# anonymousauthors001/SGS-GNN

Hardware: AMD Instinct MI355X
Metric: sampled edges/sec + training steps/sec, Reddit hybrid 20% sparsity (higher is better)
Workload: dtype f32

## Files before the change

include/sgs_hip.h:

```cpp
#ifndef SGS_HIP_H_
#define SGS_HIP_H_

#include <stddef.h>
#include <stdint.h>

#ifdef __cplusplus
extern "C" {
#endif

#define SGS_ABI_VERSION 1

#define SGS_OK 0
#define SGS_EINVAL (-1)
#define SGS_EWORKSPACE (-2)
#define SGS_EHIP (-3)

typedef void* sgs_stream_t;

int sgs_abi_version(void);
const char* sgs_last_error(void);

int sgs_rng_set_epoch_buffer(const uint64_t* epoch_dev);
int sgs_exp_noise(uint64_t seed, uint64_t stream_id, int64_t E, float* noise, sgs_stream_t stream);
int sgs_dropout_keep(uint64_t seed, uint32_t site, int64_t rows, int64_t cols, float p, uint8_t* keep,
// ... 365 lines not shown
                      const int64_t* edge_index, float* dw, void* ws, size_t ws_bytes, sgs_stream_t stream);
int sgs_cheb_spmm(int64_t K, const float* X, int64_t ldx, int64_t N, int64_t D, int64_t nnz, const int32_t* ptr, const int32_t* col,
                  const float* val, float alpha, const float* add, int64_t ldadd, const float* sub, int64_t ldsub, const float* bias, int act,
                  float p_drop, uint64_t seed, uint32_t site, float* Y, int64_t ldy, float* Y2, int64_t ldy2, float scale2,
                  sgs_stream_t stream);

size_t sgs_gemm_tn_workspace_bytes(int64_t K, int64_t M, int64_t N);
int sgs_gemm_tn(const float* A, const float* B, int64_t K, int64_t M, int64_t N, float* C, void* ws, size_t ws_bytes,
                sgs_stream_t stream);
void sgs_gemm_tn_set_tall_variant(int variant);
int sgs_gemm_tn_can_colsum(int64_t K, int64_t M, int64_t N);
int sgs_gemm_tn_colsum(const float* A, const float* B, int64_t K, int64_t M, int64_t N, float* C, float* colsum_A, void* ws,
                       size_t ws_bytes, sgs_stream_t stream);
int sgs_gemm_tn_ld(const float* A, const float* B, int64_t K, int64_t M, int64_t N, float* C, int64_t ldc, float* colsum_A, void* ws,
                   size_t ws_bytes, sgs_stream_t stream);

int sgs_er_weight(const int64_t* edge_index, int64_t E, int64_t N, const int32_t* out_ptr, const int32_t* out_dst, int walk_lengths,
                  int walks, uint64_t seed, float* weight, sgs_stream_t stream);

int sgs_adam_max_tensors(void);
int sgs_adam_step(const int64_t* desc_host, int64_t n_tensors, float lr, float beta1, float beta2, float eps, float weight_decay,
                  int maximize, uint32_t* ticket, sgs_stream_t stream);
int sgs_adam_multi_max_tensors(void);
int sgs_adam_step_multi(const int64_t* desc_host, const float* hyper_host, int64_t n_tensors, uint32_t* ticket, float* loss_sum, const float* loss,
                        uint64_t* epoch, sgs_stream_t stream);

size_t sgs_sample_topq_multi_workspace_bytes(int64_t E, int64_t D);
int sgs_sample_topq_multi(int mode, const float* p, const float* prior, double degree_bias_coef, const float* noise, uint64_t seed,
                          uint64_t stream_id0, int64_t D, int64_t E, int64_t q, const int64_t* edge_index, uint8_t* mask, int64_t* sampled_eid,
                          int64_t* sampled_edge_index, float* stats, float* st_weights, void* ws, size_t ws_bytes, sgs_stream_t stream);
// ... 35 lines not shown
```

sgs-gnn_amd/csrc/gemm_tn.hip:

```cpp
#include "sgs_common.h"

namespace sgs {
namespace {

using f32x16 = __attribute__((ext_vector_type(16))) float;
constexpr int kUnroll = 8;

__global__ void __launch_bounds__(64) gemm_tn_tile(const float* __restrict__ A, const float* __restrict__ B, int64_t K, int M, int N,
                                                  int ksplit, float* __restrict__ slab) {
    const int lane = threadIdx.x, kh = lane >> 5, l31 = lane & 31;
    const int ti = blockIdx.x, tj = blockIdx.y, s = blockIdx.z;
    const int i = ti * 32 + l31, j = tj * 32 + l31;
    const bool iok = i < M, jok = j < N;
    const int64_t per = ((K + ksplit - 1) / ksplit + 1) & ~int64_t(1);
    const int64_t k0 = s * per, k1 = (k0 + per < K) ? k0 + per : K;
    f32x16 acc;
#pragma unroll
    for (int r = 0; r < 16; ++r) acc[r] = 0.f;
    int64_t k = k0;
    for (; k + 2 * kUnroll <= k1; k += 2 * kUnroll) {
        float a[kUnroll], b[kUnroll];
#pragma unroll
        for (int u = 0; u < kUnroll; ++u) {
            const int64_t kk = k + 2 * u + kh;
// ... 9 lines not shown
        const float b = (jok && kk < k1) ? B[kk * N + j] : 0.f;
        acc = __builtin_amdgcn_mfma_f32_32x32x2f32(a, b, acc, 0, 0, 0);
    }
    float* out = slab + static_cast<int64_t>(s) * M * N;
    if (jok) {
#pragma unroll
        for (int r = 0; r < 16; ++r) {
            const int row = ti * 32 + (r & 3) + 8 * (r >> 2) + 4 * kh;
            if (row < M) out[static_cast<int64_t>(row) * N + j] = acc[r];
        }
    }
}

constexpr int kWgUnroll = 8;
template <int NW>
__global__ void __launch_bounds__(64 * NW) gemm_tn_wg(const float* __restrict__ A, const float* __restrict__ B, int64_t K, int M, int N,
                                                     float* __restrict__ C, int64_t ldc) {
    __shared__ float red[NW][16][64];
    const int lane = threadIdx.x & 63, s = threadIdx.x >> 6, kh = lane >> 5, l31 = lane & 31;
    const int ti = blockIdx.x, tj = blockIdx.y;
    const int i = ti * 32 + l31, j = tj * 32 + l31;
    const bool iok = i < M, jok = j < N;
    const int64_t per = ((K + NW - 1) / NW + 1) & ~int64_t(1);
    const int64_t k0 = s * per, k1 = (k0 + per < K) ? k0 + per : K;
    f32x16 acc;
#pragma unroll
    for (int r = 0; r < 16; ++r) acc[r] = 0.f;
    int64_t k = k0;
    for (; k + 2 * kWgUnroll <= k1; k += 2 * kWgUnroll) {
        float a[kWgUnroll], b[kWgUnroll];
#pragma unroll
        for (int u = 0; u < kWgUnroll; ++u) {
            const int64_t kk = k + 2 * u + kh;
            a[u] = iok ? A[kk * M + i] : 0.f;
            b[u] = jok ? B[kk * N + j] : 0.f;
// ... 9 lines not shown
    }
#pragma unroll
    for (int r = 0; r < 16; ++r) red[s][r][lane] = acc[r];
    __syncthreads();
    if (!jok) return;
    constexpr int RPW = 16 / NW;
#pragma unroll
    for (int q = 0; q < RPW; ++q) {
        const int r = s * RPW + q;
        float sum = 0.f;
#pragma unroll
        for (int z = 0; z < NW; ++z) sum += red[z][r][lane];
        const int row = ti * 32 + (r & 3) + 8 * (r >> 2) + 4 * kh;
        if (row < M) C[static_cast<int64_t>(row) * ldc + j] = sum;
    }
}

__global__ void __launch_bounds__(256) gemm_tn_reduce(const float* __restrict__ slab, int64_t mn, int ksplit, float* __restrict__ C,
                                                      const float* __restrict__ cpart = nullptr, int M = 0, float* __restrict__ colsum = nullptr,
                                                      int N = 0, int64_t ldc = 0, const float* __restrict__ rowscale = nullptr,
                                                      float scale = 1.f, const float* __restrict__ dzpart = nullptr, int nz = 0,
                                                      float* __restrict__ dzsum = nullptr, float* __restrict__ Craw = nullptr,
                                                      float* __restrict__ csraw = nullptr, int csplit = 0) {
    const int64_t i = static_cast<int64_t>(blockIdx.x) * 256 + threadIdx.x;
    if (i >= mn) {
        const int64_t c = i - mn;
        if (dzsum && c == M) {
            float acc = 0.f;
            for (int z = 0; z < nz; ++z) acc += dzpart[z];
            dzsum[0] = acc;
// ... 643 lines not shown
inline int pick_ksplit_tall(int64_t K, int64_t M, int64_t N) {
    const int64_t tiles = cdiv(M, 128) * cdiv(N, 64);
    int ks = 1;
    while (ks < 512 && tiles * ks < 1024 && K / (ks * 2) >= 256) ks *= 2;
    return ks;
}

inline int pick_ksplit(int64_t K, int64_t M, int64_t N) {
    if (use_tall(K, M, N)) return pick_ksplit_tall(K, M, N);
    const int64_t tiles = cdiv(M, 32) * cdiv(N, 32);
    int ks = 1;
    while (ks < 64 && tiles * ks < 1024 && K / (ks * 2) >= 64) ks *= 2;
    return ks;
}

}
}

using namespace sgs;

extern "C" {

size_t sgs_gemm_tn_workspace_bytes(int64_t K, int64_t M, int64_t N) {
    if (K < 0 || M < 0 || N < 0) return 256;
    const size_t ks = static_cast<size_t>(pick_ksplit(K, M, N));
    return carve_bytes(ks * M * N, 4) + carve_bytes(ks * M, 4) + carve_bytes(kMaskfeatMaxSlabs * 8 * M + kMaskfeatMaxSlabs, 4) + 512;
}

static int gemm_tn_impl(const float* A, const float* B, int64_t K, int64_t M, int64_t N, float* C, float* colsum_A, void* ws,
                        size_t ws_bytes, hipStream_t stream, int64_t ldc = 0, const uint32_t* Abits = nullptr, const float* dz = nullptr,
// ... 176 lines not shown
        static bool raised = false;
        if (!raised) {
            SGS_HIP_OK(hipFuncSetAttribute(reinterpret_cast<const void*>(&gemm_tn_tall_bf16x6<NW>), hipFuncAttributeMaxDynamicSharedMemorySize,
                                           static_cast<int>(lds)));
            raised = true;
        }
        n_slabs = ks / NW;
        hipLaunchKernelGGL((gemm_tn_tall_bf16x6<NW>), dim3(cdiv(M, 128), cdiv(N, 64), n_slabs), dim3(64 * NW), lds, stream, A, B, K,
                           static_cast<int>(M), static_cast<int>(N), ks, slab, colsum_A ? cpart : static_cast<float*>(nullptr));
    } else if (use_tall(K, M, N) && g_tall_bf16x6)
        hipLaunchKernelGGL((gemm_tn_tall_bf16x6<1>), dim3(cdiv(M, 128), cdiv(N, 64), ks), dim3(64), 0, stream, A, B, K, static_cast<int>(M),
                           static_cast<int>(N), ks, dst, colsum_A ? cpart : static_cast<float*>(nullptr));
    else if (use_tall(K, M, N))
        hipLaunchKernelGGL(gemm_tn_tall_tile, dim3(cdiv(M, 128), cdiv(N, 64), ks), dim3(64), 0, stream, A, B, K, static_cast<int>(M),
                           static_cast<int>(N), ks, dst, colsum_A ? cpart : static_cast<float*>(nullptr));
    else if (ks == 2 || ks == 4 || ks == 8) {
        const dim3 grid(cdiv(M, 32), cdiv(N, 32));
        const int64_t ld = ldc > 0 ? ldc : N;
        if (ks == 8 && K >= 512)
            hipLaunchKernelGGL((gemm_tn_wg<16>), grid, dim3(1024), 0, stream, A, B, K, static_cast<int>(M), static_cast<int>(N), C, ld);
        else if (ks == 8) hipLaunchKernelGGL((gemm_tn_wg<8>), grid, dim3(512), 0, stream, A, B, K, static_cast<int>(M), static_cast<int>(N), C, ld);
        else if (ks == 4) hipLaunchKernelGGL((gemm_tn_wg<4>), grid, dim3(256), 0, stream, A, B, K, static_cast<int>(M), static_cast<int>(N), C, ld);
        else              hipLaunchKernelGGL((gemm_tn_wg<2>), grid, dim3(128), 0, stream, A, B, K, static_cast<int>(M), static_cast<int>(N), C, ld);
        SGS_LAUNCH_OK();
        return SGS_OK;
    } else
        hipLaunchKernelGGL(gemm_tn_tile, dim3(cdiv(M, 32), cdiv(N, 32), ks), dim3(64), 0, stream, A, B, K, static_cast<int>(M),
                           static_cast<int>(N), ks, dst);
    if (ks > 1 || strided)
        hipLaunchKernelGGL(gemm_tn_reduce, dim3(cdiv(M * N + (colsum_A ? M : 0), 256)), dim3(256), 0, stream, slab, M * N, n_slabs, C,
                           static_cast<const float*>(colsum_A ? cpart : nullptr), static_cast<int>(M), colsum_A, static_cast<int>(N), ldc);
    SGS_LAUNCH_OK();
    return SGS_OK;
}

}
```

sgs-gnn_amd/ops.py:

```python
from __future__ import annotations

import os

import numpy as np
import torch

from . import _lib

SAMPLE_LEARNED, SAMPLE_PRIOR = 0, 1
ACT_NONE, ACT_RELU, ACT_RELU_DROPOUT = 0, 1, 2

_workspaces = {}
_retired_workspaces = []
_pin_workspaces = False


def _need_gpu(*tensors):
    for t in tensors:
        if t is not None and not t.is_cuda:
            raise RuntimeError("sgs_gnn_amd: the SGS hot path runs only on a HIP device (got a CPU tensor); "
                               "there is no CPU fallback")


def _ptr(t, dtype=None):
# ... 88 lines not shown

def memo_scope() -> int:
    return _memo_scope


def new_memo_scope() -> int:
    global _memo_scope
    _memo_scope += 1
    return _memo_scope


def drop_memos(module) -> None:
    for mod in module.modules():
        if getattr(mod, "_lin_cache", None) is not None:
            mod._lin_cache = None


_rng_epoch = None


def set_rng_epoch_buffer(epoch) -> None:
    global _rng_epoch
    L = _lib.lib()
    if epoch is not None:
        _need_gpu(epoch)
        if epoch.dtype != torch.int64 or epoch.numel() != 1:
            raise RuntimeError("sgs_gnn_amd: the RNG epoch buffer is one int64 device word")
    _lib.check(L.sgs_rng_set_epoch_buffer(None if epoch is None else epoch.data_ptr()), "sgs_rng_set_epoch_buffer")
    _rng_epoch = epoch

# ... 602 lines not shown
                       "sgs_gemm_tn_ld")
            db1 = _colsum(dv)
        dw2 = _colsum(hdz)
        db2 = _colsum(dz.view(n, 1)).reshape(1)
        if H % 4 == 0:
            dcodes = torch.empty(N, H, dtype=torch.float32, device=dev)
            dU = torch.empty(N, H, dtype=torch.float32, device=dev)
            _lib.check(L.sgs_endpoint_reduce_pair(_ptr(dfeat), _ptr(dv), _ptr(codes), N, H, graph.n_edges, _ptr(graph.in_ptr), _ptr(graph.in_src),
                                                  _ptr(graph.in_eid), _ptr(graph.out_ptr), _ptr(graph.out_dst), _ptr(graph.out_eid),
                                                  _ptr(dcodes), _ptr(dU), _stream()), "sgs_endpoint_reduce_pair")
        else:
            dcodes = _endpoint_reduce(dfeat, dfeat, codes, graph, 1.0, 1.0, H)
            dU = _endpoint_reduce(dv, dv, None, graph, 1.0, -1.0, H)
        if ctx.needs_input_grad[0]:
            dcodes.addmm_(dU, W1[:, H:])
        wsb = workspace(L.sgs_gemm_tn_workspace_bytes(N, H, H), dev)
        _lib.check(L.sgs_gemm_tn_ld(_ptr(dU), _ptr(codes), N, H, H, dW1.data_ptr() + 4 * H, 2 * H, None, wsb.data_ptr(), wsb.numel(), _stream()),
                   "sgs_gemm_tn_ld")
        return dcodes, dW1, db1, dw2, db2, None, None, None, None, None, None, None, None


def _variant_overrides_are_default() -> bool:
    L = _lib.lib()
    return L.sgs_edge_score_get_variant() < 0 and L.sgs_edge_score_get_bwd_variant() < 0


def _edge_score_backward_mask(ctx, L, codes, U, W1, b1, w2, b2, edge_index, eid, graph, n, gp_act, kept=()):
    N, H = codes.shape
    E = edge_index.shape[1]
    dev = codes.device
    f32 = dict(dtype=torch.float32, device=dev)
    p = ctx.p
    bits = torch.empty(n, H // 32, dtype=torch.int32, device=dev)
# ... 25 lines not shown
    scale = float(np.float32(1.0) / (np.float32(1.0) - np.float32(p)))
    wsg = workspace(L.sgs_gemm_tn_workspace_bytes(n, H, H), dev)
    db2 = torch.empty(1, **f32)
    _lib.check((L.sgs_gemm_tn_mask_bf16 if bf16 else L.sgs_gemm_tn_mask)(_ptr(bits), _ptr(dz), _ptr(w2), scale, _ptr(feat), n, H, H, _ptr(dW1), 2 * H, _ptr(db1), _ptr(db2), _ptr(Traw),
                                  _ptr(craw), wsg.data_ptr(), wsg.numel(), _stream()), "sgs_gemm_tn_mask")
    dw2 = _colsum(hdz) if hdz is not None else None
    dcodes = torch.empty(N, H, **f32)
    dU = torch.empty(N, H, **f32)
    _lib.check(L.sgs_endpoint_reduce_pair_bits(_ptr(dfeat), _ptr(bits), _ptr(dz), _ptr(w2), p, _ptr(codes), N, H, graph.n_edges, _ptr(graph.in_ptr),
                                               _ptr(graph.in_src), _ptr(graph.in_eid), _ptr(graph.out_ptr), _ptr(graph.out_dst),
                                               _ptr(graph.out_eid), _ptr(dcodes), _ptr(dU), _ptr(Rraw), _stream()), "sgs_endpoint_reduce_pair_bits")
    if dw2 is None:
        dw2 = torch.empty(H, **f32)
        _lib.check(L.sgs_edge_score_dw2_from_parts(_ptr(W1), _ptr(Traw), _ptr(U), _ptr(Rraw), _ptr(b1), _ptr(craw), N, H, p, _ptr(dw2), _stream()),
                   "sgs_edge_score_dw2_from_parts")
    return _edge_score_backward_mask_tail(L, codes, W1, dcodes, dU, dW1, db1, dw2, db2)


def _edge_score_backward_fused(ctx, L, codes, U, W1, b1, w2, edge_index, eid, graph, n, gp_act, kept, bits, dz):
    N, H = codes.shape
    E = edge_index.shape[1]
    dev = codes.device
    f32 = dict(dtype=torch.float32, device=dev)
    p = ctx.p
    maskbits, p_out = kept
    sd = torch.empty(n, 2, dtype=torch.int32, device=dev)
    wsd = workspace(L.sgs_edge_score_workspace_bytes(0, H, 0), dev)
    bf16 = getattr(ctx, "bf16", False)
    _lib.check((L.sgs_edge_score_bwd_prep_sd_pack_bf16 if bf16 else L.sgs_edge_score_bwd_prep_sd_pack)(_ptr(codes), N, H, _ptr(edge_index), E, _ptr(eid), n, _ptr(gp_act), _ptr(p_out), _ptr(maskbits),
                                                 _ptr(dz), _ptr(bits), _ptr(sd), _ptr(W1), _ptr(w2), p, wsd.data_ptr(), wsd.numel(), _stream()),
               "sgs_edge_score_bwd_prep_sd_pack")
# ... 3 lines not shown
                                                       wsd.numel(), _stream()), "sgs_edge_score_bwd_dfeat_fused_packed")
    dW1 = torch.empty_like(W1)
    db1, db2 = torch.empty(H, **f32), torch.empty(1, **f32)
    Traw, craw, Rraw = torch.empty(H, H, **f32), torch.empty(H, **f32), torch.empty(N, H, **f32)
    scale = float(np.float32(1.0) / (np.float32(1.0) - np.float32(p)))
    wsg = workspace(L.sgs_gemm_tn_workspace_bytes(n, H, H), dev)
    _lib.check((L.sgs_gemm_tn_mask_gather_bf16 if bf16 else L.sgs_gemm_tn_mask_gather)(_ptr(bits), _ptr(dz), _ptr(w2), scale, _ptr(codes), N, _ptr(sd), n, H, H, _ptr(dW1), 2 * H, _ptr(db1), _ptr(db2),
                                         _ptr(Traw), _ptr(craw), wsg.data_ptr(), wsg.numel(), _stream()), "sgs_gemm_tn_mask_gather")
    dcodes, dU = torch.empty(N, H, **f32), torch.empty(N, H, **f32)
    _lib.check(L.sgs_edge_score_bwd_reduce_fused(_ptr(G), _ptr(opart), _ptr(bits), _ptr(dz), _ptr(w2), p, N, H, graph.n_edges, _ptr(graph.in_ptr),
                                                 _ptr(graph.in_eid), _ptr(graph.out_ptr), _ptr(dcodes), _ptr(dU), _ptr(Rraw), _stream()),
               "sgs_edge_score_bwd_reduce_fused")
    dw2 = torch.empty(H, **f32)
    _lib.check(L.sgs_edge_score_dw2_from_parts(_ptr(W1), _ptr(Traw), _ptr(U), _ptr(Rraw), _ptr(b1), _ptr(craw), N, H, p, _ptr(dw2), _stream()),
               "sgs_edge_score_dw2_from_parts")
    return _edge_score_backward_mask_tail(L, codes, W1, dcodes, dU, dW1, db1, dw2, db2)


def _edge_score_backward_mask_tail(L, codes, W1, dcodes, dU, dW1, db1, dw2, db2):
    N, H = codes.shape
    dcodes.addmm_(dU, W1[:, H:])
    wsb = workspace(L.sgs_gemm_tn_workspace_bytes(N, H, H), codes.device)
    _lib.check(L.sgs_gemm_tn_ld(_ptr(dU), _ptr(codes), N, H, H, dW1.data_ptr() + 4 * H, 2 * H, None, wsb.data_ptr(), wsb.numel(), _stream()),
               "sgs_gemm_tn_ld")
    return dcodes, dW1, db1, dw2, db2, None, None, None, None, None, None, None, None


_EdgeScore._backward_mask = staticmethod(_edge_score_backward_mask)


def edge_score(codes, fc1_w, fc1_b, fc2_w, fc2_b, edge_index, active=None, p=0.0, seed=0, site=0, edge_id_offset=0, pairs="cached",
               precision=None):
    precision = _precision if precision is None else check_precision(precision)
    _need_gpu(codes, fc1_w, edge_index)
    if isinstance(pairs, str):
        pairs = get_pairs(edge_index, codes.shape[0])
    return _EdgeScore.apply(codes.contiguous(), fc1_w.contiguous(), fc1_b.contiguous(), fc2_w.reshape(-1).contiguous(), fc2_b.contiguous(),
                            edge_index.contiguous(), active, float(p), int(seed), int(site), int(edge_id_offset), pairs, precision)

# ... 731 lines not shown

    @staticmethod
    def forward(ctx, x, W):
        ctx.save_for_backward(x, W)
        return x @ W.t()

    @staticmethod
    def backward(ctx, dY):
        L = _lib.lib()
        x, W = ctx.saved_tensors
        dx = dW = None
        dY = dY.contiguous()
        if ctx.needs_input_grad[0]:
            dx = dY @ W
        if ctx.needs_input_grad[1]:
            K, M, N = x.shape[0], W.shape[0], W.shape[1]
            dW = torch.empty(M, N, dtype=torch.float32, device=x.device)
            ws = workspace(L.sgs_gemm_tn_workspace_bytes(K, M, N), x.device)
            _lib.check(L.sgs_gemm_tn(_ptr(dY, torch.float32), _ptr(x.contiguous(), torch.float32), K, M, N, _ptr(dW), ws.data_ptr(),
                                     ws.numel(), _stream()), "sgs_gemm_tn")
        return dx, dW


def linear_nobias(x, W):
    _need_gpu(x, W)
    return _LinearNoBias.apply(x, W)


def mean_norm(graph: Graph) -> Norm:
    L = _lib.lib()
    dev = graph.edge_index.device
    nm = Norm()
    nm.graph, nm.w, nm.handle, nm.dis, nm.loopw, nm.what_loop = graph, None, None, None, None, None
    ne = max(graph.n_edges, 1)
    nm.what_in = torch.empty(ne, dtype=torch.float32, device=dev)
# ... 77 lines not shown
    try:
        x._sgs_fcsr = (fc, x._version)
    except Exception:
        pass
    return fc


def _x_wt(x, W):
    fc = feature_csr(x)
    if fc is None:
        return x @ W.t()
    Wt = W.t().contiguous()
    return _spmm(Wt, fc.ptr, fc.col, fc.val, None, None, ACT_NONE, 0.0, 0, 0, fc.N, W.shape[0], fc.nnz)


def _dyt_x(dY, x, W_shape):
    L = _lib.lib()
    fc = feature_csr(x)
    M, Nn = W_shape
    if fc is not None:
        dWt = _spmm(dY.contiguous(), fc.tptr, fc.trow, fc.tval, None, None, ACT_NONE, 0.0, 0, 0, fc.F, M, fc.nnz)
        return dWt.t().contiguous()
    K = x.shape[0]
    dW = torch.empty(M, Nn, dtype=torch.float32, device=x.device)
    ws = workspace(L.sgs_gemm_tn_workspace_bytes(K, M, Nn), x.device)
    _lib.check(L.sgs_gemm_tn(_ptr(dY, torch.float32), _ptr(x.contiguous(), torch.float32), K, M, Nn, _ptr(dW), ws.data_ptr(), ws.numel(), _stream()),
               "sgs_gemm_tn")
    return dW


class _GCNLayer(torch.autograd.Function):

    @staticmethod
    def forward(ctx, x, W, handle, bias, nm, act, p, seed, site, xl):
        gr = nm.graph
        if xl is None:
            xl = _x_wt(x, W)
        N, D = xl.shape
        Y = _spmm(xl, gr.in_ptr, gr.in_src, nm.what_in, nm.what_loop, bias, act, p, seed, site, N, D, gr.n_edges)
        ctx.nm, ctx.act, ctx.p = nm, act, p
        ctx.has_bias, ctx.has_handle = bias is not None, handle is not None
        ctx.save_for_backward(x, W, xl, Y if act != ACT_NONE else None)
        ctx.mark_non_differentiable(xl)
# ... 8 lines not shown
        N, D = xl.shape
        dY = dY.contiguous()
        dx = dW = g = dbias = None
        want_db = ctx.has_bias and ctx.needs_input_grad[3]
        if ctx.act != ACT_NONE and want_db:
            dZ, dbias = _act_bwd_colsum(dY, Y, ctx.act, ctx.p)
        elif ctx.act != ACT_NONE:
            dZ = torch.empty_like(dY)
            _lib.check(L.sgs_act_bwd(_ptr(dY), _ptr(Y), dY.numel(), ctx.act, float(ctx.p), _ptr(dZ), _stream()), "sgs_act_bwd")
        else:
            dZ = dY
        need_x, need_W = ctx.needs_input_grad[0], ctx.needs_input_grad[1]
        if need_x or need_W:
            dxl = _spmm(dZ, gr.out_ptr, gr.out_dst, nm.what_out, nm.what_loop, None, ACT_NONE, 0.0, 0, 0, N, D, gr.n_edges)
            if need_W:
                dW = _dyt_x(dxl, x, W.shape)
            if need_x:
                dx = dxl @ W
        if ctx.has_handle and ctx.needs_input_grad[2]:
            g = torch.empty(gr.n_edges + gr.N, dtype=torch.float32, device=dY.device)
            gw, gl = g[:gr.n_edges], g[gr.n_edges:]
            _lib.check(L.sgs_sddmm_csr(_ptr(dZ), _ptr(xl), N, D, gr.n_edges, _ptr(gr.in_ptr), _ptr(gr.in_src), _ptr(gr.in_eid),
                                       gw.data_ptr(), gl.data_ptr(), _stream()), "sgs_sddmm_csr")
        if want_db and dbias is None:
            dbias = _colsum(dZ)
        return dx, dW, (_handle_grad(nm, g) if g is not None else None), dbias, None, None, None, None, None, None


def gcn_layer(x, W, bias, nm: Norm, act=ACT_NONE, p=0.0, seed=0, site=0, xl=None):
    _need_gpu(x, W, bias)
    if x.dtype != torch.float32 or x.dim() != 2 or x.shape[0] != nm.graph.N:
# ... 54 lines not shown
            return gg

        want_1 = need_x or need_W1 or need_b1 or need_g
        dxl2 = dZ1 = None
        if want_1 or need_W2:
            dxl2 = torch.empty(N, C, **f32)
            if ctx.fused:
                dZ1 = torch.empty(N, H, **f32) if want_1 else None
                db2 = torch.empty(C, **f32) if need_b2 else None
                _lib.check(L.sgs_spmm_csr_bwd_prev(_ptr(dZ2), N, C, gr.n_edges, _ptr(gr.out_ptr), _ptr(gr.out_dst), _ptr(nm.what_out),
                                                   _ptr(nm.what_loop), _ptr(W2 if want_1 else None, torch.float32), H, _ptr(h), ctx.act,
                                                   float(ctx.p), _ptr(dxl2), _ptr(dZ1), _ptr(db2), _stream()), "sgs_spmm_csr_bwd_prev")
            else:
                dxl2 = _spmm(dZ2, gr.out_ptr, gr.out_dst, nm.what_out, nm.what_loop, None, ACT_NONE, 0.0, 0, 0, N, C, gr.n_edges)
        if need_W2:
            dW2 = _dyt_x(dxl2, h, W2.shape)
        if want_1 and not ctx.fused:
            dZ1h = dxl2 @ W2
            if need_b1:
                dZ1, db1 = _act_bwd_colsum(dZ1h, h, ctx.act, ctx.p)
            else:
                dZ1 = torch.empty_like(dZ1h)
                _lib.check(L.sgs_act_bwd(_ptr(dZ1h), _ptr(h), dZ1h.numel(), ctx.act, float(ctx.p), _ptr(dZ1), _stream()), "sgs_act_bwd")
        g2 = sddmm(dZ2, xl2, C) if need_g else None
        if need_b2 and db2 is None:
            db2 = _colsum(dZ2)
        if need_x or need_W1 or (need_b1 and db1 is None and ctx.fused):
            if ctx.fused:
                dxl1 = torch.empty(N, H, **f32)
                db1 = torch.empty(H, **f32) if need_b1 else None
                _lib.check(L.sgs_spmm_csr_bwd_prev(_ptr(dZ1), N, H, gr.n_edges, _ptr(gr.out_ptr), _ptr(gr.out_dst), _ptr(nm.what_out),
                                                   _ptr(nm.what_loop), None, 0, None, ACT_NONE, 0.0, _ptr(dxl1), None, _ptr(db1), _stream()),
                           "sgs_spmm_csr_bwd_prev")
            else:
                dxl1 = _spmm(dZ1, gr.out_ptr, gr.out_dst, nm.what_out, nm.what_loop, None, ACT_NONE, 0.0, 0, 0, N, H, gr.n_edges)
            if need_W1:
                dW1 = _dyt_x(dxl1, x, W1.shape)
            if need_x:
                dx = dxl1 @ W1
        g1 = sddmm(dZ1, xl1, H) if need_g else None
        if need_b1 and db1 is None:
            db1 = _colsum(dZ1)
        if need_g:
            r2, r1 = _handle_grad(nm, g2), _handle_grad(nm, g1)
            g = r2 if r1 is None else (r1 if r2 is None else r2 + r1)
        return dx, dW1, db1, dW2, db2, g, None, None, None, None, None, None


def gcn2(x, W1, b1, W2, b2, nm: Norm, act=ACT_RELU, p=0.0, seed=0, site=0, xl1=None):
    _need_gpu(x, W1, b1, W2, b2)
    if x.dtype != torch.float32 or x.dim() != 2 or x.shape[0] != nm.graph.N:
        raise RuntimeError("gcn2: x must be float32 [N, F]")
# ... 481 lines not shown
```

sgs-gnn_amd/stepgraph.py:

```python
from __future__ import annotations

import ctypes
import gc
import os
import time

import torch

from . import _lib, ops
from .data import Batch

_DEBUG = os.environ.get("SGS_SG_DEBUG", "")
_PREFETCH = os.environ.get("SGS_SG_PREFETCH", "1") != "0"
_E_ALIGN = 2048


def _capturable(opt) -> bool:
    return all(bool(g.get("capturable", False)) for g in opt.param_groups)


def _opt_signature(optimizers):
    if optimizers is None:
        return None
    sig = []
# ... 392 lines not shown
            cur.wait_stream(self.stream)
            torch.cuda.synchronize()
            ops.workspace_handover(self.device)
            self.capture_seconds += time.perf_counter() - t0
            self.captures += 1
            if was_enabled:
                gc.enable()

    def _warm_up(self, slot: _Slot) -> None:
        from .training import _ce, learned_loss, sampled_forward
        b, a = slot.batch, self.args
        ops.drop_memos(self.model)
        ops.new_memo_scope()
        with torch.cuda.stream(self.stream):
            if not slot.sampled:
                _ce(self.criterion, self.model(b, b.edge_index), b).backward()
            else:
                st = sampled_forward(self.pipeline, a, self.model, b, self.q, self.use_checkpoint)
                if st.random_out is not None:
                    _ce(self.criterion, st.random_out, b).backward(retain_graph=True)
                    self._clear_grads()
                learned_loss(a, self.criterion, st, b).backward()
        self._clear_grads()
        torch.cuda.synchronize()

    def _capture_segments(self, c: _Slot) -> None:
        from .training import _ce, learned_loss, sampled_forward, sampled_prefix
        if not self._epoch_started:
            self.epoch_word.fill_(1)
            self.host_epoch = 1
            self._epoch_started = True
        a, batch = self.args, c.batch
        self._clear_grads()
        torch.cuda.synchronize()
        c.g1 = torch.cuda.CUDAGraph()
        ops.drop_memos(self.model)
        ops.new_memo_scope()
        if self.dp and self.g3 is None:
            self._capture_g3()
        if not c.sampled:
            if self.dp:
                self._bind_bucket()
            with torch.cuda.graph(c.g1, stream=self.stream, capture_error_mode=self.capture_mode):
                if self.dp:
                    self.sync.flat.zero_()
                out = self.model(batch, batch.edge_index)
                c.loss = _ce(self.criterion, out, batch)
                c.loss.backward(gradient=self.one)
                self._steps_and_tick((self.optimizers[1],) if (self.optimizers is not None and not self.dp) else (), c.loss)
            c.grads = self._grads()
            c.loss = c.loss.detach()
            self._clear_grads()
            return
        pre, pool = None, None
        if (a.conditional or a.sparse_edge_mlp) and _DEBUG != "fork":
            c.g0 = torch.cuda.CUDAGraph()
            ops.set_rng_epoch_buffer(self.epoch_pre)
            try:
                with ops.workspace_slot(1), torch.cuda.graph(c.g0, stream=self.stream, capture_error_mode=self.capture_mode):
                    pre = sampled_prefix(a, batch, self.q)
            finally:
                ops.set_rng_epoch_buffer(self.epoch_word)
            pool = c.g0.pool()
# ... 3 lines not shown
                                 prefix=pre, gate_publish=(self.epoch_word, self.host_gate))
        pool = c.g1.pool()
        c.cbuf = st.cbuf
        if self.debug_keep:
            c.keep = dict(rsei=st.rsei, eid=st.smp.eid, sampled_edge_index=st.sampled_edge_index,
                          edge_probs_full=st.edge_probs_full.detach(), w=st.edge_probs_for_loss.detach(),
                          learned_out=st.learned_out.detach(),
                          random_out=None if st.random_out is None else st.random_out.detach())
        c.g2l = torch.cuda.CUDAGraph()
        if self.dp:
            self._bind_bucket()
        with torch.cuda.graph(c.g2l, stream=self.stream, pool=pool, capture_error_mode=self.capture_mode):
            if self.dp:
                self.sync.flat.zero_()
            loss_l = learned_loss(a, self.criterion, st, batch)
            loss_l.backward(gradient=self.one, retain_graph=st.random_out is not None)
            if self.dp:
                self.sync.flag.fill_(1.0)
            self._steps_and_tick(tuple(self.optimizers) if (self.optimizers is not None and not self.dp) else (), loss_l)
        c.grads_l = self._grads()
        c.loss_l = loss_l.detach()
        self._clear_grads()
        c.g2r = None
        if st.random_out is not None:
            c.g2r = torch.cuda.CUDAGraph()
            if self.dp:
                self._bind_bucket()
            with torch.cuda.graph(c.g2r, stream=self.stream, pool=pool, capture_error_mode=self.capture_mode):
                if self.dp:
                    self.sync.flat.zero_()
                loss_r = _ce(self.criterion, st.random_out, batch)
                loss_r.backward(gradient=self.one)
                self._steps_and_tick((self.optimizers[1],) if (self.optimizers is not None and not self.dp) else (), loss_r)
            c.grads_r = self._grads()
            c.loss_r = loss_r.detach()
            self._clear_grads()

    def _steps_and_tick(self, opts, loss) -> None:
        from .optim import FusedAdam
        if opts and all(isinstance(o, FusedAdam) for o in opts):
            FusedAdam.step_many(opts, tick=(self.loss_sum, loss, self.epoch_word))
            return
        for o in opts:
            o.step()
        ops.loss_tick(self.loss_sum, loss, self.epoch_word)

    def _set_grads(self, grads):
# ... 210 lines not shown
```

sgs-gnn_amd/training.py:

```python
from __future__ import annotations

import torch
import torch.nn as nn

from . import ops
from .dist import GradSync, is_parallel
from .sampling import draw_learned, draw_prior, random_edge_sampling
from .utils import segment

_PIPELINES = ("two_pass", "straight_through", "hybrid")


def _fused_ce_ok(criterion) -> bool:
    return (type(criterion) is nn.CrossEntropyLoss and criterion.weight is None and criterion.reduction == "mean"
            and criterion.ignore_index == -100 and getattr(criterion, "label_smoothing", 0.0) == 0.0)


def _ce(criterion, out, batch):
    if _fused_ce_ok(criterion):
        return ops.masked_cross_entropy(out, batch.y, batch.train_mask)
    return criterion(out[batch.train_mask], batch.y[batch.train_mask])


def _backward(model, loss):
    with segment(model, "backward"):
        loss.backward()


def _has_train_nodes(batch) -> bool:
    flag = getattr(batch, "_sgs_has_train", None)
    if flag is None:
        flag = bool(batch.train_mask.any())
        try:
            batch._sgs_has_train = flag
        except Exception:
            pass
    return flag


class SampledForward:
# ... 393 lines not shown
```

Before: 98.82 million.

## Defer weight-gradient GEMMs in backward and launch them as one grouped kernel

Adds a context manager that walks the autograd graph, queues weight-gradient TN GEMMs for leaf parameters during backward, and flushes them at the end through a new grouped HIP kernel that maps a flat tile index to problem descriptors. It aims to cut per-GEMM launch overhead and fill the GPU better with many small weight-grad GEMMs run together. The cost is delayed gradient materialisation, which relies on autograd passing the allocated buffer through as .grad unchanged, plus graph-walking Python overhead at capture time. Since the steps are CUDA-graph captured, launch overhead is already partly amortised.

```diff
diff --git a/include/sgs_hip.h b/include/sgs_hip.h
--- a/include/sgs_hip.h
+++ b/include/sgs_hip.h
@@ -403,6 +403,17 @@
                        size_t ws_bytes, sgs_stream_t stream);
 int sgs_gemm_tn_ld(const float* A, const float* B, int64_t K, int64_t M, int64_t N, float* C, int64_t ldc, float* colsum_A, void* ws,
                    size_t ws_bytes, sgs_stream_t stream);
+typedef struct SgsGemmTnProblem {
+    const float* A;
+    const float* B;
+    int64_t K, M, N;
+    float* C;
+    int64_t ldc;
+    void* ws;
+    size_t ws_bytes;
+} SgsGemmTnProblem;
+int sgs_gemm_tn_group_supported(int64_t K, int64_t M, int64_t N);
+int sgs_gemm_tn_group(const SgsGemmTnProblem* problems, int count, sgs_stream_t stream);
 
 int sgs_er_weight(const int64_t* edge_index, int64_t E, int64_t N, const int32_t* out_ptr, const int32_t* out_dst, int walk_lengths,
                   int walks, uint64_t seed, float* weight, sgs_stream_t stream);
diff --git a/sgs-gnn_amd/csrc/gemm_tn.hip b/sgs-gnn_amd/csrc/gemm_tn.hip
--- a/sgs-gnn_amd/csrc/gemm_tn.hip
+++ b/sgs-gnn_amd/csrc/gemm_tn.hip
@@ -47,11 +47,10 @@
 
 constexpr int kWgUnroll = 8;
 template <int NW>
-__global__ void __launch_bounds__(64 * NW) gemm_tn_wg(const float* __restrict__ A, const float* __restrict__ B, int64_t K, int M, int N,
-                                                     float* __restrict__ C, int64_t ldc) {
+__device__ __forceinline__ void gemm_tn_wg_tile(const float* __restrict__ A, const float* __restrict__ B, int64_t K, int M, int N,
+                                                float* __restrict__ C, int64_t ldc, int ti, int tj) {
     __shared__ float red[NW][16][64];
     const int lane = threadIdx.x & 63, s = threadIdx.x >> 6, kh = lane >> 5, l31 = lane & 31;
-    const int ti = blockIdx.x, tj = blockIdx.y;
     const int i = ti * 32 + l31, j = tj * 32 + l31;
     const bool iok = i < M, jok = j < N;
     const int64_t per = ((K + NW - 1) / NW + 1) & ~int64_t(1);
@@ -91,6 +90,37 @@
         const int row = ti * 32 + (r & 3) + 8 * (r >> 2) + 4 * kh;
         if (row < M) C[static_cast<int64_t>(row) * ldc + j] = sum;
     }
+}
+
+template <int NW>
+__global__ void __launch_bounds__(64 * NW) gemm_tn_wg(const float* __restrict__ A, const float* __restrict__ B, int64_t K, int M, int N,
+                                                     float* __restrict__ C, int64_t ldc) {
+    gemm_tn_wg_tile<NW>(A, B, K, M, N, C, ldc, blockIdx.x, blockIdx.y);
+}
+
+constexpr int kGroupMax = 8;
+struct GemmTnDesc {
+    const float* A;
+    const float* B;
+    float* C;
+    int64_t K, ldc;
+    int M, N;
+    int first_tile, tiles_i;
+};
+struct GemmTnGroupArgs {
+    GemmTnDesc d[kGroupMax];
+    int count;
+};
+
+template <int NW>
+__global__ void __launch_bounds__(64 * NW) gemm_tn_wg_group(GemmTnGroupArgs a) {
+    const int t = static_cast<int>(blockIdx.x);
+    int pi = 0;
+    while (pi + 1 < a.count && t >= a.d[pi + 1].first_tile) ++pi;
+    const GemmTnDesc& d = a.d[pi];
+    const int local = t - d.first_tile;
+    const int tj = local / d.tiles_i, ti = local - tj * d.tiles_i;
+    gemm_tn_wg_tile<NW>(d.A, d.B, d.K, d.M, d.N, d.C, d.ldc, ti, tj);
 }
 
 __global__ void __launch_bounds__(256) gemm_tn_reduce(const float* __restrict__ slab, int64_t mn, int ksplit, float* __restrict__ C,
@@ -764,6 +794,13 @@
     return ks;
 }
 
+inline int wg_waves(int64_t K, int64_t M, int64_t N) {
+    if (K <= 0 || M <= 0 || N <= 0 || use_tall(K, M, N)) return 0;
+    const int ks = pick_ksplit(K, M, N);
+    if (ks == 8 && K >= 512) return 16;
+    return (ks == 2 || ks == 4 || ks == 8) ? ks : 0;
+}
+
 }
 }
 
@@ -970,13 +1007,12 @@
     else if (use_tall(K, M, N))
         hipLaunchKernelGGL(gemm_tn_tall_tile, dim3(cdiv(M, 128), cdiv(N, 64), ks), dim3(64), 0, stream, A, B, K, static_cast<int>(M),
                            static_cast<int>(N), ks, dst, colsum_A ? cpart : static_cast<float*>(nullptr));
-    else if (ks == 2 || ks == 4 || ks == 8) {
+    else if (const int nw = wg_waves(K, M, N)) {
         const dim3 grid(cdiv(M, 32), cdiv(N, 32));
         const int64_t ld = ldc > 0 ? ldc : N;
-        if (ks == 8 && K >= 512)
-            hipLaunchKernelGGL((gemm_tn_wg<16>), grid, dim3(1024), 0, stream, A, B, K, static_cast<int>(M), static_cast<int>(N), C, ld);
-        else if (ks == 8) hipLaunchKernelGGL((gemm_tn_wg<8>), grid, dim3(512), 0, stream, A, B, K, static_cast<int>(M), static_cast<int>(N), C, ld);
-        else if (ks == 4) hipLaunchKernelGGL((gemm_tn_wg<4>), grid, dim3(256), 0, stream, A, B, K, static_cast<int>(M), static_cast<int>(N), C, ld);
+        if (nw == 16)     hipLaunchKernelGGL((gemm_tn_wg<16>), grid, dim3(1024), 0, stream, A, B, K, static_cast<int>(M), static_cast<int>(N), C, ld);
+        else if (nw == 8) hipLaunchKernelGGL((gemm_tn_wg<8>), grid, dim3(512), 0, stream, A, B, K, static_cast<int>(M), static_cast<int>(N), C, ld);
+        else if (nw == 4) hipLaunchKernelGGL((gemm_tn_wg<4>), grid, dim3(256), 0, stream, A, B, K, static_cast<int>(M), static_cast<int>(N), C, ld);
         else              hipLaunchKernelGGL((gemm_tn_wg<2>), grid, dim3(128), 0, stream, A, B, K, static_cast<int>(M), static_cast<int>(N), C, ld);
         SGS_LAUNCH_OK();
         return SGS_OK;
@@ -990,4 +1026,54 @@
     return SGS_OK;
 }
 
-}
+int sgs_gemm_tn_group_supported(int64_t K, int64_t M, int64_t N) { return wg_waves(K, M, N); }
+
+int sgs_gemm_tn_group(const SgsGemmTnProblem* problems, int count, sgs_stream_t stream_) {
+    hipStream_t stream = static_cast<hipStream_t>(stream_);
+    SGS_REQUIRE(count >= 0 && (count == 0 || problems), SGS_EINVAL, "sgs_gemm_tn_group: bad problem list");
+    for (int p = 0; p < count; ++p) {
+        const SgsGemmTnProblem& q = problems[p];
+        SGS_REQUIRE(q.K >= 0 && q.M >= 0 && q.N >= 0 && q.M < (1 << 30) && q.N < (1 << 30), SGS_EINVAL, "sgs_gemm_tn_group: bad sizes");
+        SGS_REQUIRE(q.ldc == 0 || q.ldc >= q.N, SGS_EINVAL, "sgs_gemm_tn_group: ldc < N");
+        SGS_REQUIRE(q.M == 0 || q.N == 0 || (q.C && (q.K == 0 || (q.A && q.B))), SGS_EINVAL, "sgs_gemm_tn_group: null pointer");
+    }
+    for (int nw = 16; nw >= 2; nw >>= 1) {
+        GemmTnGroupArgs a;
+        a.count = 0;
+        int tiles = 0;
+        auto flush = [&]() {
+            if (a.count == 0) return;
+            for (int z = a.count; z < kGroupMax; ++z) a.d[z] = a.d[0];
+            const dim3 grid(static_cast<unsigned>(tiles));
+            if (nw == 16)     hipLaunchKernelGGL((gemm_tn_wg_group<16>), grid, dim3(1024), 0, stream, a);
+            else if (nw == 8) hipLaunchKernelGGL((gemm_tn_wg_group<8>), grid, dim3(512), 0, stream, a);
+            else if (nw == 4) hipLaunchKernelGGL((gemm_tn_wg_group<4>), grid, dim3(256), 0, stream, a);
+            else              hipLaunchKernelGGL((gemm_tn_wg_group<2>), grid, dim3(128), 0, stream, a);
+            a.count = 0;
+            tiles = 0;
+        };
+        for (int p = 0; p < count; ++p) {
+            const SgsGemmTnProblem& q = problems[p];
+            if (wg_waves(q.K, q.M, q.N) != nw) continue;
+            GemmTnDesc& d = a.d[a.count++];
+            d.A = q.A; d.B = q.B; d.C = q.C;
+            d.K = q.K; d.ldc = q.ldc > 0 ? q.ldc : q.N;
+            d.M = static_cast<int>(q.M); d.N = static_cast<int>(q.N);
+            d.first_tile = tiles;
+            d.tiles_i = static_cast<int>(cdiv(q.M, 32));
+            tiles += d.tiles_i * static_cast<int>(cdiv(q.N, 32));
+            if (a.count == kGroupMax) flush();
+        }
+        flush();
+    }
+    SGS_LAUNCH_OK();
+    for (int p = 0; p < count; ++p) {
+        const SgsGemmTnProblem& q = problems[p];
+        if (wg_waves(q.K, q.M, q.N) != 0) continue;
+        const int rc = gemm_tn_impl(q.A, q.B, q.K, q.M, q.N, q.C, nullptr, q.ws, q.ws_bytes, stream, q.ldc);
+        if (rc != SGS_OK) return rc;
+    }
+    return SGS_OK;
+}
+
+}
diff --git a/sgs-gnn_amd/ops.py b/sgs-gnn_amd/ops.py
--- a/sgs-gnn_amd/ops.py
+++ b/sgs-gnn_amd/ops.py
@@ -1,5 +1,6 @@
 from __future__ import annotations
 
+import ctypes
 import os
 
 import numpy as np
@@ -126,6 +127,109 @@
     for mod in module.modules():
         if getattr(mod, "_lin_cache", None) is not None:
             mod._lin_cache = None
+
+
+GEMM_TN_LAUNCHES = {"single": 0, "group": 0}
+_defer = None
+_defer_enabled = True
+
+
+def set_deferred_weight_grads(on: bool) -> None:
+    global _defer_enabled
+    _defer_enabled = bool(on)
+
+
+class deferred_weight_grads:
+
+    def __init__(self, *roots):
+        self.roots = roots
+        self.producers, self.queue, self.armed, self.prev = {}, [], False, None
+
+    def __enter__(self):
+        global _defer
+        self.prev = _defer
+        if not _defer_enabled:
+            return self
+        seen, stack = set(), [r.grad_fn for r in self.roots if r.grad_fn is not None]
+        prod = self.producers = {}
+        while stack:
+            fn = stack.pop()
+            if fn in seen:
+                continue
+            seen.add(fn)
+            for nxt, _ in fn.next_functions:
+                if nxt is None:
+                    continue
+                if hasattr(nxt, "variable"):
+                    prod[nxt] = prod.get(nxt, 0) + 1
+                else:
+                    stack.append(nxt)
+        self.queue, self.armed = [], False
+        self.prev, _defer = _defer, self
+        return self
+
+    def __exit__(self, *exc):
+        global _defer
+        _defer = self.prev
+        pending = len(self.queue)
+        self.queue, self.producers, self.armed = [], {}, False
+        if pending and exc[0] is None:
+            raise RuntimeError("sgs_gnn_amd: deferred weight gradients were queued but the backward pass ended without flushing them")
+        return False
+
+    def _leaf_slot_ok(self, ctx, slot):
+        node = ctx.next_functions[slot][0]
+        if node is None or self.producers.get(node) != 1:
+            return None
+        p = node.variable
+        if p.grad is not None or getattr(p, "_backward_hooks", None) or getattr(p, "_post_accumulate_grad_hooks", None):
+            return None
+        return node
+
+    def _enqueue(self, node, dY, x, grad, c_ptr, K, M, N, ldc):
+        if not self.armed:
+            torch.autograd.Variable._execution_engine.queue_callback(self._flush)
+            self.armed = True
+        self.queue.append((node, dY, x, grad.data_ptr(), c_ptr, K, M, N, ldc, grad.device.index))
+
+    def _flush(self):
+        q, self.queue, self.armed = self.queue, [], False
+        if not q:
+            return
+        L = _lib.lib()
+        for node, _, _, base, *_ in q:
+            g = node.variable.grad
+            if g is None or g.data_ptr() != base:
+                raise RuntimeError("sgs_gnn_amd: a deferred weight gradient did not become its parameter's .grad as it was (the values "
+                                   "autograd passed on were read before they were written)")
+        words = []
+        for _, dY, x, _, c_ptr, K, M, N, ldc, _ in q:
+            words += [dY.data_ptr(), x.data_ptr(), K, M, N, c_ptr, ldc, 0, 0]
+        arr = (ctypes.c_int64 * len(words))(*words)
+        dev = q[0][9]
+        stream = _raw_stream(dev) if _raw_stream is not None else torch.cuda.current_stream(dev).cuda_stream
+        GEMM_TN_LAUNCHES["group"] += 1
+        _lib.check(L.sgs_gemm_tn_group(arr, len(q), stream), "sgs_gemm_tn_group")
+
+
+def _leaf_dw(dY, x, K, M, N, leaf=None, out=None, col0=0):
+    L = _lib.lib()
+    dW = out if out is not None else torch.empty(M, N, dtype=torch.float32, device=x.device)
+    ldc = dW.shape[1]
+    c_ptr = _ptr(dW) + 4 * col0
+    dY_p, x_p = _ptr(dY, torch.float32), _ptr(x, torch.float32)
+    if _defer is not None and leaf is not None and L.sgs_gemm_tn_group_supported(K, M, N) > 0:
+        node = _defer._leaf_slot_ok(*leaf)
+        if node is not None:
+            _defer._enqueue(node, dY, x, dW, c_ptr, K, M, N, ldc)
+            return dW
+    ws = workspace(L.sgs_gemm_tn_workspace_bytes(K, M, N), x.device)
+    GEMM_TN_LAUNCHES["single"] += 1
+    if out is None:
+        _lib.check(L.sgs_gemm_tn(dY_p, x_p, K, M, N, c_ptr, ws.data_ptr(), ws.numel(), _stream()), "sgs_gemm_tn")
+    else:
+        _lib.check(L.sgs_gemm_tn_ld(dY_p, x_p, K, M, N, c_ptr, ldc, None, ws.data_ptr(), ws.numel(), _stream()), "sgs_gemm_tn_ld")
+    return dW
 
 
 _rng_epoch = None
@@ -758,9 +862,7 @@
             dU = _endpoint_reduce(dv, dv, None, graph, 1.0, -1.0, H)
         if ctx.needs_input_grad[0]:
             dcodes.addmm_(dU, W1[:, H:])
-        wsb = workspace(L.sgs_gemm_tn_workspace_bytes(N, H, H), dev)
-        _lib.check(L.sgs_gemm_tn_ld(_ptr(dU), _ptr(codes), N, H, H, dW1.data_ptr() + 4 * H, 2 * H, None, wsb.data_ptr(), wsb.numel(), _stream()),
-                   "sgs_gemm_tn_ld")
+        _leaf_dw(dU, codes, N, H, H, leaf=(ctx, 1), out=dW1, col0=H)
         return dcodes, dW1, db1, dw2, db2, None, None, None, None, None, None, None, None
 
 
@@ -816,7 +918,7 @@
         dw2 = torch.empty(H, **f32)
         _lib.check(L.sgs_edge_score_dw2_from_parts(_ptr(W1), _ptr(Traw), _ptr(U), _ptr(Rraw), _ptr(b1), _ptr(craw), N, H, p, _ptr(dw2), _stream()),
                    "sgs_edge_score_dw2_from_parts")
-    return _edge_score_backward_mask_tail(L, codes, W1, dcodes, dU, dW1, db1, dw2, db2)
+    return _edge_score_backward_mask_tail(ctx, L, codes, W1, dcodes, dU, dW1, db1, dw2, db2)
 
 
 def _edge_score_backward_fused(ctx, L, codes, U, W1, b1, w2, edge_index, eid, graph, n, gp_act, kept, bits, dz):
@@ -850,15 +952,13 @@
     dw2 = torch.empty(H, **f32)
     _lib.check(L.sgs_edge_score_dw2_from_parts(_ptr(W1), _ptr(Traw), _ptr(U), _ptr(Rraw), _ptr(b1), _ptr(craw), N, H, p, _ptr(dw2), _stream()),
                "sgs_edge_score_dw2_from_parts")
-    return _edge_score_backward_mask_tail(L, codes, W1, dcodes, dU, dW1, db1, dw2, db2)
-
-
-def _edge_score_backward_mask_tail(L, codes, W1, dcodes, dU, dW1, db1, dw2, db2):
+    return _edge_score_backward_mask_tail(ctx, L, codes, W1, dcodes, dU, dW1, db1, dw2, db2)
+
+
+def _edge_score_backward_mask_tail(ctx, L, codes, W1, dcodes, dU, dW1, db1, dw2, db2):
     N, H = codes.shape
     dcodes.addmm_(dU, W1[:, H:])
-    wsb = workspace(L.sgs_gemm_tn_workspace_bytes(N, H, H), codes.device)
-    _lib.check(L.sgs_gemm_tn_ld(_ptr(dU), _ptr(codes), N, H, H, dW1.data_ptr() + 4 * H, 2 * H, None, wsb.data_ptr(), wsb.numel(), _stream()),
-               "sgs_gemm_tn_ld")
+    _leaf_dw(dU, codes, N, H, H, leaf=(ctx, 1), out=dW1, col0=H)
     return dcodes, dW1, db1, dw2, db2, None, None, None, None, None, None, None, None
 
 
@@ -1620,11 +1720,7 @@
         if ctx.needs_input_grad[0]:
             dx = dY @ W
         if ctx.needs_input_grad[1]:
-            K, M, N = x.shape[0], W.shape[0], W.shape[1]
-            dW = torch.empty(M, N, dtype=torch.float32, device=x.device)
-            ws = workspace(L.sgs_gemm_tn_workspace_bytes(K, M, N), x.device)
-            _lib.check(L.sgs_gemm_tn(_ptr(dY, torch.float32), _ptr(x.contiguous(), torch.float32), K, M, N, _ptr(dW), ws.data_ptr(),
-                                     ws.numel(), _stream()), "sgs_gemm_tn")
+            dW = _leaf_dw(dY, x.contiguous(), x.shape[0], W.shape[0], W.shape[1], leaf=(ctx, 1))
         return dx, dW
 
 
@@ -1732,19 +1828,13 @@
     return _spmm(Wt, fc.ptr, fc.col, fc.val, None, None, ACT_NONE, 0.0, 0, 0, fc.N, W.shape[0], fc.nnz)
 
 
-def _dyt_x(dY, x, W_shape):
-    L = _lib.lib()
+def _dyt_x(dY, x, W_shape, leaf=None):
     fc = feature_csr(x)
     M, Nn = W_shape
     if fc is not None:
         dWt = _spmm(dY.contiguous(), fc.tptr, fc.trow, fc.tval, None, None, ACT_NONE, 0.0, 0, 0, fc.F, M, fc.nnz)
         return dWt.t().contiguous()
-    K = x.shape[0]
-    dW = torch.empty(M, Nn, dtype=torch.float32, device=x.device)
-    ws = workspace(L.sgs_gemm_tn_workspace_bytes(K, M, Nn), x.device)
-    _lib.check(L.sgs_gemm_tn(_ptr(dY, torch.float32), _ptr(x.contiguous(), torch.float32), K, M, Nn, _ptr(dW), ws.data_ptr(), ws.numel(), _stream()),
-               "sgs_gemm_tn")
-    return dW
+    return _leaf_dw(dY, x.contiguous(), x.shape[0], M, Nn, leaf=leaf)
 
 
 class _GCNLayer(torch.autograd.Function):
@@ -1783,7 +1873,7 @@
         if need_x or need_W:
             dxl = _spmm(dZ, gr.out_ptr, gr.out_dst, nm.what_out, nm.what_loop, None, ACT_NONE, 0.0, 0, 0, N, D, gr.n_edges)
             if need_W:
-                dW = _dyt_x(dxl, x, W.shape)
+                dW = _dyt_x(dxl, x, W.shape, leaf=(ctx, 1))
             if need_x:
                 dx = dxl @ W
         if ctx.has_handle and ctx.needs_input_grad[2]:
@@ -1868,7 +1958,7 @@
             else:
                 dxl2 = _spmm(dZ2, gr.out_ptr, gr.out_dst, nm.what_out, nm.what_loop, None, ACT_NONE, 0.0, 0, 0, N, C, gr.n_edges)
         if need_W2:
-            dW2 = _dyt_x(dxl2, h, W2.shape)
+            dW2 = _dyt_x(dxl2, h, W2.shape, leaf=(ctx, 3))
         if want_1 and not ctx.fused:
             dZ1h = dxl2 @ W2
             if need_b1:
@@ -1889,7 +1979,7 @@
             else:
                 dxl1 = _spmm(dZ1, gr.out_ptr, gr.out_dst, nm.what_out, nm.what_loop, None, ACT_NONE, 0.0, 0, 0, N, H, gr.n_edges)
             if need_W1:
-                dW1 = _dyt_x(dxl1, x, W1.shape)
+                dW1 = _dyt_x(dxl1, x, W1.shape, leaf=(ctx, 1))
             if need_x:
                 dx = dxl1 @ W1
         g1 = sddmm(dZ1, xl1, H) if need_g else None
diff --git a/sgs-gnn_amd/stepgraph.py b/sgs-gnn_amd/stepgraph.py
--- a/sgs-gnn_amd/stepgraph.py
+++ b/sgs-gnn_amd/stepgraph.py
@@ -430,13 +430,19 @@
         ops.new_memo_scope()
         with torch.cuda.stream(self.stream):
             if not slot.sampled:
-                _ce(self.criterion, self.model(b, b.edge_index), b).backward()
+                loss = _ce(self.criterion, self.model(b, b.edge_index), b)
+                with ops.deferred_weight_grads(loss):
+                    loss.backward()
             else:
                 st = sampled_forward(self.pipeline, a, self.model, b, self.q, self.use_checkpoint)
                 if st.random_out is not None:
-                    _ce(self.criterion, st.random_out, b).backward(retain_graph=True)
+                    loss = _ce(self.criterion, st.random_out, b)
+                    with ops.deferred_weight_grads(loss):
+                        loss.backward(retain_graph=True)
                     self._clear_grads()
-                learned_loss(a, self.criterion, st, b).backward()
+                loss = learned_loss(a, self.criterion, st, b)
+                with ops.deferred_weight_grads(loss):
+                    loss.backward()
         self._clear_grads()
         torch.cuda.synchronize()
 
@@ -462,7 +468,8 @@
                     self.sync.flat.zero_()
                 out = self.model(batch, batch.edge_index)
                 c.loss = _ce(self.criterion, out, batch)
-                c.loss.backward(gradient=self.one)
+                with ops.deferred_weight_grads(c.loss):
+                    c.loss.backward(gradient=self.one)
                 self._steps_and_tick((self.optimizers[1],) if (self.optimizers is not None and not self.dp) else (), c.loss)
             c.grads = self._grads()
             c.loss = c.loss.detach()
@@ -496,7 +503,8 @@
             if self.dp:
                 self.sync.flat.zero_()
             loss_l = learned_loss(a, self.criterion, st, batch)
-            loss_l.backward(gradient=self.one, retain_graph=st.random_out is not None)
+            with ops.deferred_weight_grads(loss_l):
+                loss_l.backward(gradient=self.one, retain_graph=st.random_out is not None)
             if self.dp:
                 self.sync.flag.fill_(1.0)
             self._steps_and_tick(tuple(self.optimizers) if (self.optimizers is not None and not self.dp) else (), loss_l)
@@ -512,7 +520,8 @@
                 if self.dp:
                     self.sync.flat.zero_()
                 loss_r = _ce(self.criterion, st.random_out, batch)
-                loss_r.backward(gradient=self.one)
+                with ops.deferred_weight_grads(loss_r):
+                    loss_r.backward(gradient=self.one)
                 self._steps_and_tick((self.optimizers[1],) if (self.optimizers is not None and not self.dp) else (), loss_r)
             c.grads_r = self._grads()
             c.loss_r = loss_r.detach()
diff --git a/sgs-gnn_amd/training.py b/sgs-gnn_amd/training.py
--- a/sgs-gnn_amd/training.py
+++ b/sgs-gnn_amd/training.py
@@ -23,7 +23,7 @@
 
 
 def _backward(model, loss):
-    with segment(model, "backward"):
+    with segment(model, "backward"), ops.deferred_weight_grads(loss):
         loss.backward()
 
 
```

Measured after the change: 103.7 million, median of 6. 4.9% higher.
